# OpenDriveLab/ST-P3

Hardware: AMD Instinct MI355X
Metric: BEV samples/sec (6-cam x 3-frame fwd+bwd) (higher is better)
Workload: dtype bf16 convs / f32 voxel pool; 1 GPU; BASELINE configs[2]: batch=4/GPU, 6-cam 224x480, T=3, full STP3 fwd+bwd with segmentation + pedestrian + hdmap + depth CE + instance centerness/offset + flow losses, grad-clip 5, Adam; EfficientNet-B4, D=48, C=64, BEV 200x200; global_batch=4, parallelism=dp1, launch=hipgraph

## Files before the change

### st-p3_amd/csrc/stp3_dwconv.hip

```cpp
#include <hip/hip_runtime.h>
#include <mutex>
#include <vector>
#include <stdint.h>
#include <stdlib.h>

#include "stp3_cdna.h"
#include "stp3_hip.h"

namespace {

struct DwDims {
    int N, H, W, C, Ho, Wo;
    int pad_t, pad_l;
};

template <typename T> struct Vec;
template <> struct Vec<float> {
    static constexpr int N = 4;
    float4 v;
    __device__ void load(const float* p) { v = *reinterpret_cast<const float4*>(p); }
    __device__ void store(float* p) const { *reinterpret_cast<float4*>(p) = v; }
    __device__ void zero() { v = make_float4(0.f, 0.f, 0.f, 0.f); }
    __device__ void to_float(float* f) const { f[0] = v.x; f[1] = v.y; f[2] = v.z; f[3] = v.w; }
    __device__ void from_float(const float* f) { v = make_float4(f[0], f[1], f[2], f[3]); }
};
struct bf16x8 { uint4 v; };
template <> struct Vec<uint16_t> {
    static constexpr int N = 8;
    uint4 v;
    __device__ void load(const uint16_t* p) { v = *reinterpret_cast<const uint4*>(p); }
    __device__ void store(uint16_t* p) const { *reinterpret_cast<uint4*>(p) = v; }
    __device__ void zero() { v = make_uint4(0, 0, 0, 0); }
    __device__ void to_float(float* f) const {
        const uint32_t w[4] = {v.x, v.y, v.z, v.w};
#pragma unroll
        for (int i = 0; i < 4; ++i) {
            f[2 * i] = __uint_as_float(w[i] << 16);
            f[2 * i + 1] = __uint_as_float(w[i] & 0xffff0000u);
        }
    }
    __device__ void from_float(const float* f) {
        uint32_t w[4];
#pragma unroll
        for (int i = 0; i < 4; ++i) w[i] = pack_bf16(f[2 * i], f[2 * i + 1]);
        v = make_uint4(w[0], w[1], w[2], w[3]);
    }
};

template <typename T, typename Off>
__device__ __forceinline__ const T* at(const T* base, Off byte_off) {
    return reinterpret_cast<const T*>(reinterpret_cast<const char*>(base) + byte_off);
}
template <typename T, typename Off>
__device__ __forceinline__ T* at(T* base, Off byte_off) {
    return reinterpret_cast<T*>(reinterpret_cast<char*>(base) + byte_off);
}

__device__ __forceinline__ int xcd_order(int bid, int nwg) {
    const int q = nwg >> 3, r = nwg & 7, xcd = bid & 7;
    return (xcd < r ? xcd * (q + 1) : r * (q + 1) + (xcd - r) * q) + (bid >> 3);
}

template <typename T, int K, int S, int TW, bool FLIP, typename Off, bool AFFINE = false>
__global__ __launch_bounds__(256) void dwconv_fwd_kernel(DwDims d, const T* __restrict__ x,
                                                         const float* __restrict__ w, const float* __restrict__ bias,
                                                         T* __restrict__ y, const float* __restrict__ coef = nullptr,
                                                         int act = STP3_ACT_NONE) {
    constexpr int VN = Vec<T>::N;
    const int CV = d.C / VN;
    const int wgroups = (d.Wo + TW - 1) / TW;
    const Off total = (Off)d.N * d.Ho * wgroups * CV;
    const Off tid = (Off)xcd_order(blockIdx.x, gridDim.x) * 256 + threadIdx.x;
    if (tid >= total) return;
    const int cv = (int)(tid % (Off)CV);
    Off r = tid / (Off)CV;
    const int wg = (int)(r % (Off)wgroups);
    r /= (Off)wgroups;
    const int ho = (int)(r % (Off)d.Ho);
    const int n = (int)(r / (Off)d.Ho);
    const int c0 = cv * VN;
    const int wo0 = wg * TW;
    float acc[TW][VN];
#pragma unroll
    for (int i = 0; i < TW; ++i)
#pragma unroll
        for (int j = 0; j < VN; ++j) acc[i][j] = bias ? bias[c0 + j] : 0.f;
    constexpr int SPAN = (TW - 1) * S + K;
    const int wi0 = wo0 * S - d.pad_l;
    const Off pix = (Off)d.C * sizeof(T);
    const Off wtap = (Off)d.C * sizeof(float);
    const Off wc0 = (Off)c0 * sizeof(float);
#pragma unroll
    for (int kh = 0; kh < K; ++kh) {
        const int hi = ho * S + kh - d.pad_t;
        if (hi < 0 || hi >= d.H) continue;
        float wk[K][VN];
#pragma unroll
        for (int kw = 0; kw < K; ++kw) {
            const float* wp = at(w, (Off)(FLIP ? (K - 1 - kh) * K + (K - 1 - kw) : kh * K + kw) * wtap + wc0);
#pragma unroll
            for (int j = 0; j < VN; ++j) wk[kw][j] = wp[j];
        }
        const Off xrow = ((Off)(n * d.H + hi) * d.W) * pix + (Off)c0 * sizeof(T);
        float xin[SPAN][VN];
#pragma unroll
        for (int i = 0; i < SPAN; ++i) {
            const int wi = wi0 + i;
            Vec<T> v;
            if (wi >= 0 && wi < d.W) v.load(at(x, xrow + (Off)wi * pix)); else v.zero();
            v.to_float(xin[i]);
        }
#pragma unroll
        for (int o = 0; o < TW; ++o)
#pragma unroll
            for (int kw = 0; kw < K; ++kw)
#pragma unroll
                for (int j = 0; j < VN; ++j) acc[o][j] = fmaf(xin[o * S + kw][j], wk[kw][j], acc[o][j]);
    }
    const Off yrow = ((Off)(n * d.Ho + ho) * d.Wo) * pix + (Off)c0 * sizeof(T);
    float cs[VN], ct[VN];
    if (AFFINE) {
#pragma unroll
        for (int j = 0; j < VN; ++j) {
            cs[j] = coef[c0 + j];
            ct[j] = coef[d.C + c0 + j];
        }
    }
#pragma unroll
    for (int o = 0; o < TW; ++o) {
        if (wo0 + o < d.Wo) {
            Vec<T> v;
            v.from_float(acc[o]);
            if (AFFINE) {
                float t[VN];
                v.to_float(t);
#pragma unroll
                for (int j = 0; j < VN; ++j) t[j] = fmaf(t[j], cs[j], ct[j]);
                if (act == STP3_ACT_SWISH) {
#pragma unroll
                    for (int j = 0; j < VN; ++j) t[j] = t[j] * fast_sigmoid(t[j]);
                } else if (act == STP3_ACT_RELU) {
#pragma unroll
                    for (int j = 0; j < VN; ++j) t[j] = fmaxf(t[j], 0.f);
                }
                v.from_float(t);
            }
            v.store(at(y, yrow + (Off)(wo0 + o) * pix));
        }
    }
}

template <typename T, int K>
__global__ __launch_bounds__(256) void dwconv_bwd_data_s2_kernel(DwDims d, int qrows, int qcols, const T* __restrict__ dy,
                                                                 const float* __restrict__ w, T* __restrict__ dx) {
    constexpr int VN = Vec<T>::N;
    constexpr int R = (K + 1) / 2;
    constexpr bool kRegW = K == 3;
    const int CV = d.C / VN;
    const int CVB = min(CV, 256);
    const int QL = 256 / CVB;
    const int cv = blockIdx.y * CVB + threadIdx.x % CVB, ql = threadIdx.x / CVB;
    if (ql >= QL || cv >= CV) return;
    const int c0 = cv * VN;
    float wr[kRegW ? K * K : 1][VN];
    if (kRegW) {
#pragma unroll
        for (int t = 0; t < K * K; ++t)
#pragma unroll
            for (int j = 0; j < VN; ++j) wr[t][j] = w[t * d.C + c0 + j];
    }
    const int a0 = d.pad_t >> 1, b0 = d.pad_l >> 1;
    const int64_t total = (int64_t)d.N * qrows * qcols;
    for (int64_t q = (int64_t)blockIdx.x * QL + ql; q < total; q += (int64_t)gridDim.x * QL) {
        const int bi = (int)(q % qcols);
        int64_t r = q / qcols;
        const int ai = (int)(r % qrows);
        const int n = (int)(r / qrows);
        const int a = a0 + ai, b = b0 + bi;
        float acc[2][2][VN];
#pragma unroll
        for (int pr = 0; pr < 2; ++pr)
#pragma unroll
            for (int pc = 0; pc < 2; ++pc)
#pragma unroll
                for (int j = 0; j < VN; ++j) acc[pr][pc][j] = 0.f;
#pragma unroll
        for (int dr = 0; dr < R; ++dr) {
            const int ho = a - dr;
            if (ho < 0 || ho >= d.Ho) continue;
#pragma unroll
            for (int dc = 0; dc < R; ++dc) {
                const int wo = b - dc;
                if (wo < 0 || wo >= d.Wo) continue;
                Vec<T> v;
                v.load(dy + ((int64_t)(n * d.Ho + ho) * d.Wo + wo) * d.C + c0);
                float g[VN];
                v.to_float(g);
#pragma unroll
                for (int pr = 0; pr < 2; ++pr) {
                    const int kh = 2 * dr + pr;
                    if (kh >= K) continue;
#pragma unroll
                    for (int pc = 0; pc < 2; ++pc) {
                        const int kw = 2 * dc + pc;
                        if (kw >= K) continue;
                        if (kRegW) {
#pragma unroll
                            for (int j = 0; j < VN; ++j) acc[pr][pc][j] = fmaf(g[j], wr[kh * K + kw][j], acc[pr][pc][j]);
                        } else {
#pragma unroll
                            for (int j = 0; j < VN; ++j)
                                acc[pr][pc][j] = fmaf(g[j], w[(kh * K + kw) * d.C + c0 + j], acc[pr][pc][j]);
                        }
                    }
                }
            }
        }
#pragma unroll
        for (int pr = 0; pr < 2; ++pr) {
            const int hi = 2 * a + pr - d.pad_t;
            if (hi < 0 || hi >= d.H) continue;
#pragma unroll
            for (int pc = 0; pc < 2; ++pc) {
                const int wi = 2 * b + pc - d.pad_l;
                if (wi < 0 || wi >= d.W) continue;
                Vec<T> o;
                o.from_float(acc[pr][pc]);
                o.store(dx + ((int64_t)(n * d.H + hi) * d.W + wi) * d.C + c0);
            }
        }
    }
}

template <typename T, int K, int S, typename Off>
__global__ __launch_bounds__(256) void dwconv_bwd_weight_kernel(DwDims d, int nbx, const T* __restrict__ x,
                                                                const T* __restrict__ dy,
                                                                float* __restrict__ partial) {
    constexpr int VN = Vec<T>::N;
    constexpr int KK = K * K;
    constexpr int TW = 4;
    constexpr int SPAN = (TW - 1) * S + K;
    extern __shared__ __attribute__((aligned(16))) float red[];
    const int CV = d.C / VN;
    const int CVB = min(CV, 256);
    const int PL = 256 / CVB;
    const int cvb = threadIdx.x % CVB, pl = threadIdx.x / CVB;
    const int v = xcd_order(blockIdx.x, gridDim.x);
    const int kh = v % K;
    const int bxi = (v / K) % nbx, byi = v / (K * nbx);
    const int cv = byi * CVB + cvb;
    const bool live = pl < PL && cv < CV;
    const int c0 = cv * VN;
    float acc[K][VN];
#pragma unroll
    for (int t = 0; t < K; ++t)
#pragma unroll
        for (int j = 0; j < VN; ++j) acc[t][j] = 0.f;
    const int wgroups = (d.Wo + TW - 1) / TW;
    const int ngroups = d.N * d.Ho * wgroups;
    if (live) {
        for (int p = bxi * PL + pl; p < ngroups; p += nbx * PL) {
            const int wg = p % wgroups;
            const int r = p / wgroups;
            const int ho = r % d.Ho;
            const int n = r / d.Ho;
            const int hi = ho * S + kh - d.pad_t;
            if (hi < 0 || hi >= d.H) continue;
            const int wo0 = wg * TW;
            const Off pix = (Off)d.C * sizeof(T);
            const Off grow = ((Off)(n * d.Ho + ho) * d.Wo + wo0) * pix + (Off)c0 * sizeof(T);
            const Off xrow = ((Off)(n * d.H + hi) * d.W) * pix + (Off)c0 * sizeof(T);
            const int wi0 = wo0 * S - d.pad_l;
            float g[TW][VN], xin[SPAN][VN];
#pragma unroll
            for (int o = 0; o < TW; ++o) {
                Vec<T> v;
                if (wo0 + o < d.Wo) v.load(at(dy, grow + (Off)o * pix)); else v.zero();
                v.to_float(g[o]);
            }
#pragma unroll
            for (int i = 0; i < SPAN; ++i) {
                const int wi = wi0 + i;
                Vec<T> v;
                if (wi >= 0 && wi < d.W) v.load(at(x, xrow + (Off)wi * pix)); else v.zero();
                v.to_float(xin[i]);
            }
#pragma unroll
            for (int o = 0; o < TW; ++o)
#pragma unroll
                for (int kw = 0; kw < K; ++kw)
#pragma unroll
                    for (int j = 0; j < VN; ++j) acc[kw][j] = fmaf(g[o][j], xin[o * S + kw][j], acc[kw][j]);
        }
    }
    const int rowlen = CVB * VN;
    if (pl < PL) {
#pragma unroll
        for (int t = 0; t < K; ++t)
#pragma unroll
            for (int j = 0; j < VN; ++j) red[(pl * K + t) * rowlen + cvb * VN + j] = acc[t][j];
    }
    __syncthreads();
    for (int i = threadIdx.x; i < K * rowlen; i += 256) {
        const int t = i / rowlen, cc = i % rowlen;
        const int c = byi * rowlen + cc;
        if (c >= d.C) continue;
        float s = 0.f;
        for (int q = 0; q < PL; ++q) s += red[(q * K + t) * rowlen + cc];
        partial[((int64_t)bxi * KK + kh * K + t) * d.C + c] = s;
    }
}

__global__ __launch_bounds__(256) void dwconv_reduce_partials_kernel(int nblocks, int n, const float* __restrict__ partial,
                                                                     float* __restrict__ dw, int channels) {
    __shared__ float red[256];
    const int il = threadIdx.x & 63, bl = threadIdx.x >> 6;
    const int i = blockIdx.x * 64 + il;
    float s0 = 0.f, s1 = 0.f, s2 = 0.f, s3 = 0.f;
    if (i < n) {
        int b = bl;
        for (; b + 12 < nblocks; b += 16) {
            const float a = partial[(int64_t)b * n + i], c = partial[(int64_t)(b + 4) * n + i];
            const float e = partial[(int64_t)(b + 8) * n + i], f = partial[(int64_t)(b + 12) * n + i];
            s0 += a; s1 += c; s2 += e; s3 += f;
        }
        for (; b < nblocks; b += 4) s0 += partial[(int64_t)b * n + i];
    }
    red[threadIdx.x] = (s0 + s1) + (s2 + s3);
    __syncthreads();
    if (bl == 0 && i < n) {
        const int o = channels > 0 ? (i % channels) * (n / channels) + i / channels : i;
        dw[o] = (red[il] + red[64 + il]) + (red[128 + il] + red[192 + il]);
    }
}


template <typename T, int K, int S, typename Off>
__global__ __launch_bounds__(256) void dwconv_fwd_stats_kernel(DwDims d, const T* __restrict__ x, const float* __restrict__ w,
                                                               T* __restrict__ y, float* __restrict__ partial) {
    constexpr int VN = Vec<T>::N;
    constexpr int TW = 4;
    constexpr int SPAN = (TW - 1) * S + K;
    extern __shared__ __attribute__((aligned(16))) float red[];
    const int CV = d.C / VN;
    const int CVB = min(CV, 256);
    const int PL = 256 / CVB;
    const int cvb = threadIdx.x % CVB, pl = threadIdx.x / CVB;
    const int cv = blockIdx.y * CVB + cvb;
    const bool live = pl < PL && cv < CV;
    const int c0 = cv * VN;
    float s1[VN], s2[VN];
#pragma unroll
    for (int j = 0; j < VN; ++j) s1[j] = s2[j] = 0.f;
    const int wgroups = (d.Wo + TW - 1) / TW;
    const int ngroups = d.N * d.Ho * wgroups;
    if (live) {
        for (int p = blockIdx.x * PL + pl; p < ngroups; p += gridDim.x * PL) {
            const int wg = p % wgroups;
            const int r = p / wgroups;
            const int ho = r % d.Ho;
            const int n = r / d.Ho;
            const int wo0 = wg * TW;
            float acc[TW][VN];
#pragma unroll
            for (int i = 0; i < TW; ++i)
#pragma unroll
                for (int j = 0; j < VN; ++j) acc[i][j] = 0.f;
            const int wi0 = wo0 * S - d.pad_l;
            const Off pix = (Off)d.C * sizeof(T);
            const Off wtap = (Off)d.C * sizeof(float), wc0 = (Off)c0 * sizeof(float);
#pragma unroll
            for (int kh = 0; kh < K; ++kh) {
                const int hi = ho * S + kh - d.pad_t;
                if (hi < 0 || hi >= d.H) continue;
                float wk[K][VN];
#pragma unroll
                for (int kw = 0; kw < K; ++kw) {
                    const float* wp = at(w, (Off)(kh * K + kw) * wtap + wc0);
#pragma unroll
                    for (int j = 0; j < VN; ++j) wk[kw][j] = wp[j];
                }
                const Off xrow = ((Off)(n * d.H + hi) * d.W) * pix + (Off)c0 * sizeof(T);
                float xin[SPAN][VN];
#pragma unroll
                for (int i = 0; i < SPAN; ++i) {
                    const int wi = wi0 + i;
                    Vec<T> v;
                    if (wi >= 0 && wi < d.W) v.load(at(x, xrow + (Off)wi * pix)); else v.zero();
                    v.to_float(xin[i]);
                }
#pragma unroll
                for (int o = 0; o < TW; ++o)
#pragma unroll
                    for (int kw = 0; kw < K; ++kw)
#pragma unroll
                        for (int j = 0; j < VN; ++j) acc[o][j] = fmaf(xin[o * S + kw][j], wk[kw][j], acc[o][j]);
            }
            const Off yrow = ((Off)(n * d.Ho + ho) * d.Wo) * pix + (Off)c0 * sizeof(T);
#pragma unroll
            for (int o = 0; o < TW; ++o) {
                if (wo0 + o < d.Wo) {
                    Vec<T> v;
                    v.from_float(acc[o]);
                    v.store(at(y, yrow + (Off)(wo0 + o) * pix));
                    float rv[VN];
                    v.to_float(rv);
#pragma unroll
                    for (int j = 0; j < VN; ++j) {
                        s1[j] += rv[j];
                        s2[j] = fmaf(rv[j], rv[j], s2[j]);
                    }
                }
            }
        }
    }
    const int rowlen = CVB * VN;
    if (pl < PL) {
#pragma unroll
        for (int j = 0; j < VN; ++j) {
            red[(pl * 2) * rowlen + cvb * VN + j] = live ? s1[j] : 0.f;
            red[(pl * 2 + 1) * rowlen + cvb * VN + j] = live ? s2[j] : 0.f;
        }
    }
    __syncthreads();
    for (int i = threadIdx.x; i < 2 * rowlen; i += 256) {
        const int k = i / rowlen, cc = i - k * rowlen;
        const int c = blockIdx.y * rowlen + cc;
        if (c >= d.C) continue;
        float t = 0.f;
        for (int q = 0; q < PL; ++q) t += red[(q * 2 + k) * rowlen + cc];
        partial[((int64_t)blockIdx.x * 2 + k) * d.C + c] = t;
    }
}

constexpr int kRedCols = 8, kRedLanes = 256 / kRedCols;
__global__ __launch_bounds__(256) void dwconv_stat_reduce_kernel(int nblocks, int n, const float* __restrict__ partial,
                                                                 float* __restrict__ sums) {
    __shared__ double red[256];
    const int il = threadIdx.x % kRedCols, bl = threadIdx.x / kRedCols;
    const int i = blockIdx.x * kRedCols + il;
    double s0 = 0.0, s1 = 0.0, s2 = 0.0, s3 = 0.0;
    if (i < n) {
        const float* src = partial + i;
        int b = bl;
        for (; b + 3 * kRedLanes < nblocks; b += 4 * kRedLanes) {
            const float a = src[(int64_t)b * n], c = src[(int64_t)(b + kRedLanes) * n];
            const float e = src[(int64_t)(b + 2 * kRedLanes) * n], f = src[(int64_t)(b + 3 * kRedLanes) * n];
            s0 += (double)a; s1 += (double)c; s2 += (double)e; s3 += (double)f;
        }
        for (; b < nblocks; b += kRedLanes) s0 += (double)src[(int64_t)b * n];
    }
    red[threadIdx.x] = (s0 + s1) + (s2 + s3);
    __syncthreads();
    for (int st = kRedLanes / 2; st > 0; st >>= 1) {
        if (bl < st) red[threadIdx.x] += red[threadIdx.x + st * kRedCols];
        __syncthreads();
    }
    if (bl == 0 && i < n) sums[i] = (float)red[il];
}

struct BnFin {
    float inv_count, unbias, eps, momentum;
    const float* gamma;
    const float* beta;
    float* running_mean;
    float* running_var;
    float* coef;
};
__global__ __launch_bounds__(256) void dwconv_stat_reduce_finalize_kernel(int nblocks, int C, const float* __restrict__ partial,
                                                                          float* __restrict__ sums, BnFin f) {
    __shared__ double red[256];
    const int il = threadIdx.x % kRedCols, bl = threadIdx.x / kRedCols;
    const int c = blockIdx.x * (kRedCols / 2) + (il & 3), k = il >> 2;
    const int n = 2 * C;
    const int i = k * C + c;
    double s0 = 0.0, s1 = 0.0, s2 = 0.0, s3 = 0.0;
    if (c < C) {
        const float* src = partial + i;
        int b = bl;
        for (; b + 3 * kRedLanes < nblocks; b += 4 * kRedLanes) {
            const float a = src[(int64_t)b * n], cc = src[(int64_t)(b + kRedLanes) * n];
            const float e = src[(int64_t)(b + 2 * kRedLanes) * n], g = src[(int64_t)(b + 3 * kRedLanes) * n];
            s0 += (double)a; s1 += (double)cc; s2 += (double)e; s3 += (double)g;
        }
        for (; b < nblocks; b += kRedLanes) s0 += (double)src[(int64_t)b * n];
    }
    red[threadIdx.x] = (s0 + s1) + (s2 + s3);
    __syncthreads();
    for (int st = kRedLanes / 2; st > 0; st >>= 1) {
        if (bl < st) red[threadIdx.x] += red[threadIdx.x + st * kRedCols];
        __syncthreads();
    }
    if (bl == 0 && c < C) sums[i] = (float)red[il];
    if (threadIdx.x < 4 && c < C) {
        const float sum = (float)red[il], sq = (float)red[4 + il];
        const float mean = sum * f.inv_count;
        const float var = fmaxf(sq * f.inv_count - mean * mean, 0.f);
        const float invstd = 1.0f / sqrtf(var + f.eps);
        const float scale = (f.gamma ? f.gamma[c] : 1.f) * invstd;
        f.coef[c] = scale;
        f.coef[C + c] = (f.beta ? f.beta[c] : 0.f) - mean * scale;
        f.coef[2 * C + c] = mean;
        f.coef[3 * C + c] = invstd;
        if (f.running_mean) {
            f.running_mean[c] = (1.f - f.momentum) * f.running_mean[c] + f.momentum * mean;
            f.running_var[c] = (1.f - f.momentum) * f.running_var[c] + f.momentum * var * f.unbias;
        }
    }
}

constexpr int kStatBlocks = 2048;
constexpr int kWgradBlocks = 512;

template <typename Kern>
inline int resident_blocks(Kern kernel, size_t lds) {
    struct Entry { const void* fn; size_t lds; int blocks; };
    static std::mutex mu;
    static std::vector<Entry> cache;
    static int cus = 0;
    std::lock_guard<std::mutex> lock(mu);
    for (const Entry& e : cache)
        if (e.fn == (const void*)kernel && e.lds == lds) return e.blocks;
    if (cus == 0) {
        int dev = 0;
        if (hipGetDevice(&dev) != hipSuccess ||
            hipDeviceGetAttribute(&cus, hipDeviceAttributeMultiprocessorCount, dev) != hipSuccess || cus < 1)
            cus = 256;
    }
    int per_cu = 0;
    if (hipOccupancyMaxActiveBlocksPerMultiprocessor(&per_cu, kernel, 256, lds) != hipSuccess || per_cu < 1) per_cu = 1;
    cache.push_back(Entry{(const void*)kernel, lds, per_cu * cus});
    return per_cu * cus;
}

inline int status() {
    hipError_t e = hipGetLastError();
    return e == hipSuccess ? STP3_OK : -(int)e;
}

inline int check(const stp3_dwconv_dims* p, DwDims* d, int* vec) {
    if (!p) return STP3_EINVAL;
    if (p->N <= 0 || p->H <= 0 || p->W <= 0 || p->C <= 0 || p->Ho <= 0 || p->Wo <= 0) return STP3_EINVAL;
    if (!(((p->K == 3 || p->K == 5) && (p->stride == 1 || p->stride == 2)) || (p->K == 7 && p->stride == 1)))
        return STP3_EUNSUP;
    if (p->dtype != STP3_DTYPE_F32 && p->dtype != STP3_DTYPE_BF16) return STP3_EUNSUP;
    *vec = p->dtype == STP3_DTYPE_BF16 ? 8 : 4;
    if (p->C % *vec) return STP3_EUNSUP;
    if ((int64_t)p->N * p->H * p->W * p->C >= (1LL << 40)) return STP3_EUNSUP;
    d->N = p->N; d->H = p->H; d->W = p->W; d->C = p->C; d->Ho = p->Ho; d->Wo = p->Wo;
    d->pad_t = p->pad_top; d->pad_l = p->pad_left;
    return STP3_OK;
}

template <typename T>
inline bool small_tensors(const DwDims& d) {
    const uint64_t lim = (1ull << 32) - (uint64_t)(d.W + d.Wo + 16) * d.C * sizeof(float);
    return (uint64_t)d.N * d.H * d.W * d.C * sizeof(T) < lim && (uint64_t)d.N * d.Ho * d.Wo * d.C * sizeof(T) < lim &&
           (uint64_t)64 * d.C * sizeof(float) < lim;
}

template <typename T, int K, int S>
int launch_fwd(const DwDims& d, const void* x, const float* w, const float* bias, void* y, hipStream_t s) {
    constexpr int TW = 4;
    const int CV = d.C / Vec<T>::N;
    const int64_t total = (int64_t)d.N * d.Ho * ((d.Wo + TW - 1) / TW) * CV;
    if (small_tensors<T>(d))
        hipLaunchKernelGGL((dwconv_fwd_kernel<T, K, S, TW, false, uint32_t>), dim3((unsigned)((total + 255) / 256)), dim3(256), 0,
                           s, d, (const T*)x, w, bias, (T*)y, (const float*)nullptr, 0);
    else
        hipLaunchKernelGGL((dwconv_fwd_kernel<T, K, S, TW, false, uint64_t>), dim3((unsigned)((total + 255) / 256)), dim3(256), 0,
                           s, d, (const T*)x, w, bias, (T*)y, (const float*)nullptr, 0);
    return status();
}
template <int K, int S>
int launch_fwd_affine(const DwDims& d, const void* x, const float* w, const float* coef, int act, void* y, hipStream_t s) {
    typedef uint16_t T;
    constexpr int TW = 4;
    const int CV = d.C / Vec<T>::N;
    const int64_t total = (int64_t)d.N * d.Ho * ((d.Wo + TW - 1) / TW) * CV;
    if (small_tensors<T>(d))
        hipLaunchKernelGGL((dwconv_fwd_kernel<T, K, S, TW, false, uint32_t, true>), dim3((unsigned)((total + 255) / 256)), dim3(256),
                           0, s, d, (const T*)x, w, (const float*)nullptr, (T*)y, coef, act);
    else
        hipLaunchKernelGGL((dwconv_fwd_kernel<T, K, S, TW, false, uint64_t, true>), dim3((unsigned)((total + 255) / 256)), dim3(256),
                           0, s, d, (const T*)x, w, (const float*)nullptr, (T*)y, coef, act);
    return status();
}
template <typename T, int K, int S>
int launch_fwd_stats(const DwDims& d, const void* x, const float* w, void* y, float* sums, float* ws, hipStream_t s,
                     const BnFin* fin = nullptr) {
    constexpr int VN = Vec<T>::N;
    const int CV = d.C / VN;
    const int CVB = CV < 256 ? CV : 256;
    const int PL = 256 / CVB;
    const int64_t ngroups = (int64_t)d.N * d.Ho * ((d.Wo + 3) / 4);
    if (ngroups >= (1LL << 31)) return STP3_EUNSUP;
    const int by = (CV + CVB - 1) / CVB;
    int64_t want = (ngroups + PL - 1) / PL;
    const size_t lds = (size_t)PL * 2 * CVB * VN * sizeof(float);
    const bool small = small_tensors<T>(d);
    int limit = small ? resident_blocks(dwconv_fwd_stats_kernel<T, K, S, uint32_t>, lds)
                      : resident_blocks(dwconv_fwd_stats_kernel<T, K, S, uint64_t>, lds);
    if (limit > kStatBlocks) limit = kStatBlocks;
    const int cap = limit / by > 0 ? limit / by : 1;
    const int bx = (int)(want < cap ? want : cap);
    if (small)
        hipLaunchKernelGGL((dwconv_fwd_stats_kernel<T, K, S, uint32_t>), dim3(bx, by), dim3(256), lds, s, d, (const T*)x, w, (T*)y, ws);
    else
        hipLaunchKernelGGL((dwconv_fwd_stats_kernel<T, K, S, uint64_t>), dim3(bx, by), dim3(256), lds, s, d, (const T*)x, w, (T*)y, ws);
    if (fin)
        hipLaunchKernelGGL(dwconv_stat_reduce_finalize_kernel, dim3((d.C + kRedCols / 2 - 1) / (kRedCols / 2)), dim3(256), 0, s, bx,
                           d.C, ws, sums, *fin);
    else
        hipLaunchKernelGGL(dwconv_stat_reduce_kernel, dim3((2 * d.C + kRedCols - 1) / kRedCols), dim3(256), 0, s, bx, 2 * d.C, ws, sums);
    return status();
}
template <typename T, int K, int S>
int launch_bwd_data(const DwDims& d, const void* dy, const float* w, void* dx, hipStream_t s) {
    if constexpr (S == 1) {
        constexpr int TW = 4;
        DwDims f = d;
        f.H = d.Ho; f.W = d.Wo; f.Ho = d.H; f.Wo = d.W;
        f.pad_t = K - 1 - d.pad_t; f.pad_l = K - 1 - d.pad_l;
        const int64_t n = (int64_t)f.N * f.Ho * ((f.Wo + TW - 1) / TW) * (f.C / Vec<T>::N);
        if (small_tensors<T>(f))
            hipLaunchKernelGGL((dwconv_fwd_kernel<T, K, 1, TW, true, uint32_t>), dim3((unsigned)((n + 255) / 256)), dim3(256), 0, s,
                               f, (const T*)dy, w, (const float*)nullptr, (T*)dx, (const float*)nullptr, 0);
        else
            hipLaunchKernelGGL((dwconv_fwd_kernel<T, K, 1, TW, true, uint64_t>), dim3((unsigned)((n + 255) / 256)), dim3(256), 0, s,
                               f, (const T*)dy, w, (const float*)nullptr, (T*)dx, (const float*)nullptr, 0);
        return status();
    } else if constexpr (S == 2) {
        const int qrows = ((d.H - 1 + d.pad_t) >> 1) - (d.pad_t >> 1) + 1;
        const int qcols = ((d.W - 1 + d.pad_l) >> 1) - (d.pad_l >> 1) + 1;
        const int CV = d.C / Vec<T>::N;
        const int CVB = CV < 256 ? CV : 256;
        const int QL = 256 / CVB;
        const int by = (CV + CVB - 1) / CVB;
        const int64_t want = ((int64_t)d.N * qrows * qcols + QL - 1) / QL;
        int cap = resident_blocks(dwconv_bwd_data_s2_kernel<T, K>, 0) / by;
        if (cap < 1) cap = 1;
        const int bx = (int)(want < cap ? want : cap);
        hipLaunchKernelGGL((dwconv_bwd_data_s2_kernel<T, K>), dim3(bx, by), dim3(256), 0, s, d, qrows, qcols, (const T*)dy, w,
                           (T*)dx);
        return status();
    } else {
        return STP3_EUNSUP;
    }
}
template <typename T, int K, int S>
int launch_bwd_weight(const DwDims& d, const void* x, const void* dy, float* dw, float* ws, hipStream_t s, bool param_layout) {
    constexpr int VN = Vec<T>::N;
    const int CV = d.C / VN;
    const int CVB = CV < 256 ? CV : 256;
    const int PL = 256 / CVB;
    const int64_t npix = (int64_t)d.N * d.Ho * ((d.Wo + 3) / 4);
    if (npix >= (1LL << 31)) return STP3_EUNSUP;
    int64_t want = (npix + PL - 1) / PL;
    const int by = (CV + CVB - 1) / CVB;
    const size_t lds = (size_t)PL * K * CVB * VN * sizeof(float);
    const bool small = small_tensors<T>(d);
    int cap = (small ? resident_blocks(dwconv_bwd_weight_kernel<T, K, S, uint32_t>, lds)
                     : resident_blocks(dwconv_bwd_weight_kernel<T, K, S, uint64_t>, lds)) / (by * K);
    if (cap > kWgradBlocks) cap = kWgradBlocks;
    if (cap < 1) cap = 1;
    const int bx = (int)(want < cap ? want : cap);
    if (small)
        hipLaunchKernelGGL((dwconv_bwd_weight_kernel<T, K, S, uint32_t>), dim3(bx * by * K), dim3(256), lds, s, d, bx, (const T*)x,
                           (const T*)dy, ws);
    else
        hipLaunchKernelGGL((dwconv_bwd_weight_kernel<T, K, S, uint64_t>), dim3(bx * by * K), dim3(256), lds, s, d, bx, (const T*)x,
                           (const T*)dy, ws);
    const int n = K * K * d.C;
    hipLaunchKernelGGL(dwconv_reduce_partials_kernel, dim3((n + 63) / 64), dim3(256), 0, s, bx, n, ws, dw, param_layout ? d.C : 0);
    return status();
}

#define DISPATCH(FN, ...)                                                                               \
    do {                                                                                                \
        const bool bf = p->dtype == STP3_DTYPE_BF16;                                                    \
        if (p->K == 3 && p->stride == 1) return bf ? FN<uint16_t, 3, 1>(__VA_ARGS__) : FN<float, 3, 1>(__VA_ARGS__); \
        if (p->K == 3 && p->stride == 2) return bf ? FN<uint16_t, 3, 2>(__VA_ARGS__) : FN<float, 3, 2>(__VA_ARGS__); \
        if (p->K == 5 && p->stride == 1) return bf ? FN<uint16_t, 5, 1>(__VA_ARGS__) : FN<float, 5, 1>(__VA_ARGS__); \
        if (p->K == 7) return bf ? FN<uint16_t, 7, 1>(__VA_ARGS__) : FN<float, 7, 1>(__VA_ARGS__);                   \
        return bf ? FN<uint16_t, 5, 2>(__VA_ARGS__) : FN<float, 5, 2>(__VA_ARGS__);                       \
    } while (0)

}

extern "C" {

int stp3_dwconv2d_fwd(const stp3_dwconv_dims* p, const void* x, const float* w, void* y, void* stream) {
    DwDims d; int vec;
    int rc = check(p, &d, &vec);
    if (rc) return rc;
    if (!x || !w || !y) return STP3_EINVAL;
    DISPATCH(launch_fwd, d, x, w, (const float*)nullptr, y, (hipStream_t)stream);
}

int stp3_dwconv2d_fwd_bias(const stp3_dwconv_dims* p, const void* x, const float* w, const float* bias, void* y,
                           void* stream) {
    DwDims d; int vec;
    int rc = check(p, &d, &vec);
    if (rc) return rc;
    if (!x || !w || !y) return STP3_EINVAL;
    DISPATCH(launch_fwd, d, x, w, bias, y, (hipStream_t)stream);
}

int stp3_dwconv2d_fwd_affine(const stp3_dwconv_dims* p, const void* x, const float* w, const float* coef, int32_t act,
                             void* y, void* stream) {
    DwDims d; int vec;
    int rc = check(p, &d, &vec);
    if (rc) return rc;
    if (!x || !w || !coef || !y) return STP3_EINVAL;
    if (act != STP3_ACT_NONE && act != STP3_ACT_RELU && act != STP3_ACT_SWISH) return STP3_EINVAL;
    if (p->dtype != STP3_DTYPE_BF16 || p->K == 7) return STP3_EUNSUP;
    hipStream_t s = (hipStream_t)stream;
    if (p->K == 3) return p->stride == 1 ? launch_fwd_affine<3, 1>(d, x, w, coef, act, y, s) : launch_fwd_affine<3, 2>(d, x, w, coef, act, y, s);
    return p->stride == 1 ? launch_fwd_affine<5, 1>(d, x, w, coef, act, y, s) : launch_fwd_affine<5, 2>(d, x, w, coef, act, y, s);
}

int stp3_dwconv2d_fwd_stats_workspace(const stp3_dwconv_dims* p, size_t* bytes) {
    DwDims d; int vec;
    int rc = check(p, &d, &vec);
    if (rc) return rc;
    if (!bytes) return STP3_EINVAL;
    *bytes = (size_t)kStatBlocks * 2 * p->C * sizeof(float);
    return STP3_OK;
}

int stp3_dwconv2d_fwd_stats(const stp3_dwconv_dims* p, const void* x, const float* w, void* y, float* sums, void* workspace,
                            size_t workspace_bytes, void* stream) {
    DwDims d; int vec;
    int rc = check(p, &d, &vec);
    if (rc) return rc;
    if (!x || !w || !y || !sums || !workspace) return STP3_EINVAL;
    if (workspace_bytes < (size_t)kStatBlocks * 2 * p->C * sizeof(float)) return STP3_ENOSPACE;
    DISPATCH(launch_fwd_stats, d, x, w, y, sums, (float*)workspace, (hipStream_t)stream);
}

int stp3_dwconv2d_fwd_stats_bn(const stp3_dwconv_dims* p, const void* x, const float* w, void* y, float* sums, double count,
                               const float* gamma, const float* beta, float eps, float momentum, float* running_mean,
                               float* running_var, float* coef, void* workspace, size_t workspace_bytes, void* stream) {
    DwDims d; int vec;
    int rc = check(p, &d, &vec);
    if (rc) return rc;
    if (!x || !w || !y || !sums || !coef || !workspace || !(count >= 1.0)) return STP3_EINVAL;
    if ((running_mean == nullptr) != (running_var == nullptr)) return STP3_EINVAL;
    if (workspace_bytes < (size_t)kStatBlocks * 2 * p->C * sizeof(float)) return STP3_ENOSPACE;
    BnFin fin;
    fin.inv_count = (float)(1.0 / count);
    fin.unbias = count > 1.0 ? (float)(count / (count - 1.0)) : 1.f;
    fin.eps = eps; fin.momentum = momentum; fin.gamma = gamma; fin.beta = beta;
    fin.running_mean = running_mean; fin.running_var = running_var; fin.coef = coef;
    DISPATCH(launch_fwd_stats, d, x, w, y, sums, (float*)workspace, (hipStream_t)stream, &fin);
}

int stp3_dwconv2d_bwd_data(const stp3_dwconv_dims* p, const void* dy, const float* w, void* dx, void* stream) {
    DwDims d; int vec;
    int rc = check(p, &d, &vec);
    if (rc) return rc;
    if (!dy || !w || !dx) return STP3_EINVAL;
    DISPATCH(launch_bwd_data, d, dy, w, dx, (hipStream_t)stream);
}

int stp3_dwconv2d_bwd_weight_workspace(const stp3_dwconv_dims* p, size_t* bytes) {
    DwDims d; int vec;
    int rc = check(p, &d, &vec);
    if (rc) return rc;
    if (!bytes) return STP3_EINVAL;
    *bytes = (size_t)kWgradBlocks * p->K * p->K * p->C * sizeof(float);
    return STP3_OK;
}

int stp3_dwconv2d_bwd_weight(const stp3_dwconv_dims* p, const void* x, const void* dy, float* dw, void* workspace,
                             size_t workspace_bytes, void* stream) {
    DwDims d; int vec;
    int rc = check(p, &d, &vec);
    if (rc) return rc;
    if (!x || !dy || !dw || !workspace) return STP3_EINVAL;
    if (workspace_bytes < (size_t)kWgradBlocks * p->K * p->K * p->C * sizeof(float)) return STP3_ENOSPACE;
    DISPATCH(launch_bwd_weight, d, x, dy, dw, (float*)workspace, (hipStream_t)stream, false);
}

int stp3_dwconv2d_bwd_weight_oihw(const stp3_dwconv_dims* p, const void* x, const void* dy, float* dw, void* workspace,
                                  size_t workspace_bytes, void* stream) {
    DwDims d; int vec;
    int rc = check(p, &d, &vec);
    if (rc) return rc;
    if (!x || !dy || !dw || !workspace) return STP3_EINVAL;
    if (workspace_bytes < (size_t)kWgradBlocks * p->K * p->K * p->C * sizeof(float)) return STP3_ENOSPACE;
    DISPATCH(launch_bwd_weight, d, x, dy, dw, (float*)workspace, (hipStream_t)stream, true);
}

}
```

Baseline: 113.3 samples/s.

## Use buffer loads for depthwise conv and stage stride-2 bwd taps in LDS

Adds a BufAddr offset mode for tensors under 2 GiB. In it, the forward, forward-stats and weight-gradient depthwise kernels read through buffer_load16 with out-of-bounds offsets that hardware zero-fills, replacing branchy global loads and 64-bit address math. Separately, the stride-2 backward-data kernel for K>3 now stages its weights in LDS as float4 slabs and re-splits channels across the y grid instead of reading weights from global memory per tap. This adds LDS usage and a block barrier, and relies on buffer descriptor bounds being correct.

```diff
diff --git a/st-p3_amd/csrc/stp3_dwconv.hip b/st-p3_amd/csrc/stp3_dwconv.hip
--- a/st-p3_amd/csrc/stp3_dwconv.hip
+++ b/st-p3_amd/csrc/stp3_dwconv.hip
@@ -61,23 +61,49 @@
     return (xcd < r ? xcd * (q + 1) : r * (q + 1) + (xcd - r) * q) + (bid >> 3);
 }
 
+struct BufAddr {};
+template <typename Off> struct OffsetOf { typedef Off type; };
+template <> struct OffsetOf<BufAddr> { typedef uint32_t type; };
+template <typename Off> struct IsBuf { static constexpr bool value = false; };
+template <> struct IsBuf<BufAddr> { static constexpr bool value = true; };
+
+template <typename T, int SPAN, typename Off>
+__device__ __forceinline__ void load_span(float (*xin)[Vec<T>::N], const T* __restrict__ x, stp3_buffer xb,
+                                          typename OffsetOf<Off>::type xrow, typename OffsetOf<Off>::type pix, int wi0, int W) {
+    typedef typename OffsetOf<Off>::type O;
+    O off = xrow + (O)wi0 * pix;
+#pragma unroll
+    for (int i = 0; i < SPAN; ++i, off += pix) {
+        const int wi = wi0 + i;
+        Vec<T> v;
+        if constexpr (IsBuf<Off>::value) {
+            const stp3_u32x4 q = buffer_load16(xb, (unsigned)wi < (unsigned)W ? off : (O)kBufOob);
+            __builtin_memcpy(&v.v, &q, 16);
+        } else {
+            if (wi >= 0 && wi < W) v.load(at(x, off)); else v.zero();
+        }
+        v.to_float(xin[i]);
+    }
+}
+
 template <typename T, int K, int S, int TW, bool FLIP, typename Off, bool AFFINE = false>
 __global__ __launch_bounds__(256) void dwconv_fwd_kernel(DwDims d, const T* __restrict__ x,
                                                          const float* __restrict__ w, const float* __restrict__ bias,
                                                          T* __restrict__ y, const float* __restrict__ coef = nullptr,
                                                          int act = STP3_ACT_NONE) {
     constexpr int VN = Vec<T>::N;
+    typedef typename OffsetOf<Off>::type O;
     const int CV = d.C / VN;
     const int wgroups = (d.Wo + TW - 1) / TW;
-    const Off total = (Off)d.N * d.Ho * wgroups * CV;
-    const Off tid = (Off)xcd_order(blockIdx.x, gridDim.x) * 256 + threadIdx.x;
+    const O total = (O)d.N * d.Ho * wgroups * CV;
+    const O tid = (O)xcd_order(blockIdx.x, gridDim.x) * 256 + threadIdx.x;
     if (tid >= total) return;
-    const int cv = (int)(tid % (Off)CV);
-    Off r = tid / (Off)CV;
-    const int wg = (int)(r % (Off)wgroups);
-    r /= (Off)wgroups;
-    const int ho = (int)(r % (Off)d.Ho);
-    const int n = (int)(r / (Off)d.Ho);
+    const int cv = (int)(tid % (O)CV);
+    O r = tid / (O)CV;
+    const int wg = (int)(r % (O)wgroups);
+    r /= (O)wgroups;
+    const int ho = (int)(r % (O)d.Ho);
+    const int n = (int)(r / (O)d.Ho);
     const int c0 = cv * VN;
     const int wo0 = wg * TW;
     float acc[TW][VN];
@@ -87,9 +113,10 @@
         for (int j = 0; j < VN; ++j) acc[i][j] = bias ? bias[c0 + j] : 0.f;
     constexpr int SPAN = (TW - 1) * S + K;
     const int wi0 = wo0 * S - d.pad_l;
-    const Off pix = (Off)d.C * sizeof(T);
-    const Off wtap = (Off)d.C * sizeof(float);
-    const Off wc0 = (Off)c0 * sizeof(float);
+    const O pix = (O)d.C * sizeof(T);
+    const O wtap = (O)d.C * sizeof(float);
+    const O wc0 = (O)c0 * sizeof(float);
+    const stp3_buffer xb = make_buffer(x, IsBuf<Off>::value ? (uint32_t)d.N * d.H * d.W * (uint32_t)pix : 0u);
 #pragma unroll
     for (int kh = 0; kh < K; ++kh) {
         const int hi = ho * S + kh - d.pad_t;
@@ -97,19 +124,13 @@
         float wk[K][VN];
 #pragma unroll
         for (int kw = 0; kw < K; ++kw) {
-            const float* wp = at(w, (Off)(FLIP ? (K - 1 - kh) * K + (K - 1 - kw) : kh * K + kw) * wtap + wc0);
+            const float* wp = at(w, (O)(FLIP ? (K - 1 - kh) * K + (K - 1 - kw) : kh * K + kw) * wtap + wc0);
 #pragma unroll
             for (int j = 0; j < VN; ++j) wk[kw][j] = wp[j];
         }
-        const Off xrow = ((Off)(n * d.H + hi) * d.W) * pix + (Off)c0 * sizeof(T);
+        const O xrow = ((O)(n * d.H + hi) * d.W) * pix + (O)c0 * sizeof(T);
         float xin[SPAN][VN];
-#pragma unroll
-        for (int i = 0; i < SPAN; ++i) {
-            const int wi = wi0 + i;
-            Vec<T> v;
-            if (wi >= 0 && wi < d.W) v.load(at(x, xrow + (Off)wi * pix)); else v.zero();
-            v.to_float(xin[i]);
-        }
+        load_span<T, SPAN, Off>(xin, x, xb, xrow, pix, wi0, d.W);
 #pragma unroll
         for (int o = 0; o < TW; ++o)
 #pragma unroll
@@ -117,7 +138,7 @@
 #pragma unroll
                 for (int j = 0; j < VN; ++j) acc[o][j] = fmaf(xin[o * S + kw][j], wk[kw][j], acc[o][j]);
     }
-    const Off yrow = ((Off)(n * d.Ho + ho) * d.Wo) * pix + (Off)c0 * sizeof(T);
+    const O yrow = ((O)(n * d.Ho + ho) * d.Wo) * pix + (O)c0 * sizeof(T);
     float cs[VN], ct[VN];
     if (AFFINE) {
 #pragma unroll
@@ -145,22 +166,39 @@
                 }
                 v.from_float(t);
             }
-            v.store(at(y, yrow + (Off)(wo0 + o) * pix));
-        }
-    }
+            v.store(at(y, yrow + (O)(wo0 + o) * pix));
+        }
+    }
+}
+
+__host__ __device__ constexpr int quad_slab(int K) { return K == 3 ? 256 : 32; }
+
+template <int VN, int KK, int SLAB>
+__device__ __forceinline__ void stage_taps(float* tab, const float* __restrict__ w, int C, int CVB) {
+    const int cbase = blockIdx.y * CVB * VN;
+    for (int t = 0; t < KK; ++t) {
+        const float* src = w + t * C + cbase;
+        for (int cl = threadIdx.x; cl < CVB * VN; cl += 256)
+            tab[((t * (VN / 4) + (cl % VN) / 4) * SLAB + cl / VN) * 4 + (cl & 3)] = cbase + cl < C ? src[cl] : 0.f;
+    }
+    __syncthreads();
 }
 
 template <typename T, int K>
 __global__ __launch_bounds__(256) void dwconv_bwd_data_s2_kernel(DwDims d, int qrows, int qcols, const T* __restrict__ dy,
                                                                  const float* __restrict__ w, T* __restrict__ dx) {
-    constexpr int VN = Vec<T>::N;
+    constexpr int VN = Vec<T>::N, HV = VN / 4, SLAB = quad_slab(K);
     constexpr int R = (K + 1) / 2;
     constexpr bool kRegW = K == 3;
+    extern __shared__ __attribute__((aligned(16))) float taps[];
     const int CV = d.C / VN;
-    const int CVB = min(CV, 256);
+    const int CVB = (CV + gridDim.y - 1) / gridDim.y;
     const int QL = 256 / CVB;
-    const int cv = blockIdx.y * CVB + threadIdx.x % CVB, ql = threadIdx.x / CVB;
+    const int cvb = threadIdx.x % CVB;
+    const int cv = blockIdx.y * CVB + cvb, ql = threadIdx.x / CVB;
+    if (!kRegW) stage_taps<VN, K * K, SLAB>(taps, w, d.C, CVB);
     if (ql >= QL || cv >= CV) return;
+    const float4* tp = reinterpret_cast<const float4*>(taps) + cvb;
     const int c0 = cv * VN;
     float wr[kRegW ? K * K : 1][VN];
     if (kRegW) {
@@ -208,9 +246,14 @@
 #pragma unroll
                             for (int j = 0; j < VN; ++j) acc[pr][pc][j] = fmaf(g[j], wr[kh * K + kw][j], acc[pr][pc][j]);
                         } else {
-#pragma unroll
-                            for (int j = 0; j < VN; ++j)
-                                acc[pr][pc][j] = fmaf(g[j], w[(kh * K + kw) * d.C + c0 + j], acc[pr][pc][j]);
+                            float wt[VN];
+#pragma unroll
+                            for (int h = 0; h < HV; ++h) {
+                                const float4 t = tp[((kh * K + kw) * HV + h) * SLAB];
+                                wt[4 * h] = t.x; wt[4 * h + 1] = t.y; wt[4 * h + 2] = t.z; wt[4 * h + 3] = t.w;
+                            }
+#pragma unroll
+                            for (int j = 0; j < VN; ++j) acc[pr][pc][j] = fmaf(g[j], wt[j], acc[pr][pc][j]);
                         }
                     }
                 }
@@ -240,6 +283,8 @@
     constexpr int KK = K * K;
     constexpr int TW = 4;
     constexpr int SPAN = (TW - 1) * S + K;
+    constexpr bool BUF = IsBuf<Off>::value;
+    typedef typename OffsetOf<Off>::type O;
     extern __shared__ __attribute__((aligned(16))) float red[];
     const int CV = d.C / VN;
     const int CVB = min(CV, 256);
@@ -259,6 +304,9 @@
     const int wgroups = (d.Wo + TW - 1) / TW;
     const int ngroups = d.N * d.Ho * wgroups;
     if (live) {
+        const O pix = (O)d.C * sizeof(T);
+        const stp3_buffer xb = make_buffer(x, BUF ? (uint32_t)d.N * d.H * d.W * (uint32_t)pix : 0u);
+        const stp3_buffer gb = make_buffer(dy, BUF ? (uint32_t)d.N * d.Ho * d.Wo * (uint32_t)pix : 0u);
         for (int p = bxi * PL + pl; p < ngroups; p += nbx * PL) {
             const int wg = p % wgroups;
             const int r = p / wgroups;
@@ -267,22 +315,32 @@
             const int hi = ho * S + kh - d.pad_t;
             if (hi < 0 || hi >= d.H) continue;
             const int wo0 = wg * TW;
-            const Off pix = (Off)d.C * sizeof(T);
-            const Off grow = ((Off)(n * d.Ho + ho) * d.Wo + wo0) * pix + (Off)c0 * sizeof(T);
-            const Off xrow = ((Off)(n * d.H + hi) * d.W) * pix + (Off)c0 * sizeof(T);
+            const O grow = ((O)(n * d.Ho + ho) * d.Wo + wo0) * pix + (O)c0 * sizeof(T);
+            const O xrow = ((O)(n * d.H + hi) * d.W) * pix + (O)c0 * sizeof(T);
             const int wi0 = wo0 * S - d.pad_l;
             float g[TW][VN], xin[SPAN][VN];
-#pragma unroll
-            for (int o = 0; o < TW; ++o) {
+            O goff = grow, xoff = xrow + (O)wi0 * pix;
+#pragma unroll
+            for (int o = 0; o < TW; ++o, goff += pix) {
                 Vec<T> v;
-                if (wo0 + o < d.Wo) v.load(at(dy, grow + (Off)o * pix)); else v.zero();
+                if constexpr (BUF) {
+                    const stp3_u32x4 q = buffer_load16(gb, wo0 + o < d.Wo ? goff : (O)kBufOob);
+                    __builtin_memcpy(&v.v, &q, 16);
+                } else {
+                    if (wo0 + o < d.Wo) v.load(at(dy, goff)); else v.zero();
+                }
                 v.to_float(g[o]);
             }
 #pragma unroll
-            for (int i = 0; i < SPAN; ++i) {
+            for (int i = 0; i < SPAN; ++i, xoff += pix) {
                 const int wi = wi0 + i;
                 Vec<T> v;
-                if (wi >= 0 && wi < d.W) v.load(at(x, xrow + (Off)wi * pix)); else v.zero();
+                if constexpr (BUF) {
+                    const stp3_u32x4 q = buffer_load16(xb, (unsigned)wi < (unsigned)d.W ? xoff : (O)kBufOob);
+                    __builtin_memcpy(&v.v, &q, 16);
+                } else {
+                    if (wi >= 0 && wi < d.W) v.load(at(x, xoff)); else v.zero();
+                }
                 v.to_float(xin[i]);
             }
 #pragma unroll
@@ -341,6 +399,7 @@
     constexpr int VN = Vec<T>::N;
     constexpr int TW = 4;
     constexpr int SPAN = (TW - 1) * S + K;
+    typedef typename OffsetOf<Off>::type O;
     extern __shared__ __attribute__((aligned(16))) float red[];
     const int CV = d.C / VN;
     const int CVB = min(CV, 256);
@@ -355,6 +414,9 @@
     const int wgroups = (d.Wo + TW - 1) / TW;
     const int ngroups = d.N * d.Ho * wgroups;
     if (live) {
+        const O pix = (O)d.C * sizeof(T);
+        const O wtap = (O)d.C * sizeof(float), wc0 = (O)c0 * sizeof(float);
+        const stp3_buffer xb = make_buffer(x, IsBuf<Off>::value ? (uint32_t)d.N * d.H * d.W * (uint32_t)pix : 0u);
         for (int p = blockIdx.x * PL + pl; p < ngroups; p += gridDim.x * PL) {
             const int wg = p % wgroups;
             const int r = p / wgroups;
@@ -367,8 +429,6 @@
 #pragma unroll
                 for (int j = 0; j < VN; ++j) acc[i][j] = 0.f;
             const int wi0 = wo0 * S - d.pad_l;
-            const Off pix = (Off)d.C * sizeof(T);
-            const Off wtap = (Off)d.C * sizeof(float), wc0 = (Off)c0 * sizeof(float);
 #pragma unroll
             for (int kh = 0; kh < K; ++kh) {
                 const int hi = ho * S + kh - d.pad_t;
@@ -376,19 +436,13 @@
                 float wk[K][VN];
 #pragma unroll
                 for (int kw = 0; kw < K; ++kw) {
-                    const float* wp = at(w, (Off)(kh * K + kw) * wtap + wc0);
+                    const float* wp = at(w, (O)(kh * K + kw) * wtap + wc0);
 #pragma unroll
                     for (int j = 0; j < VN; ++j) wk[kw][j] = wp[j];
                 }
-                const Off xrow = ((Off)(n * d.H + hi) * d.W) * pix + (Off)c0 * sizeof(T);
+                const O xrow = ((O)(n * d.H + hi) * d.W) * pix + (O)c0 * sizeof(T);
                 float xin[SPAN][VN];
-#pragma unroll
-                for (int i = 0; i < SPAN; ++i) {
-                    const int wi = wi0 + i;
-                    Vec<T> v;
-                    if (wi >= 0 && wi < d.W) v.load(at(x, xrow + (Off)wi * pix)); else v.zero();
-                    v.to_float(xin[i]);
-                }
+                load_span<T, SPAN, Off>(xin, x, xb, xrow, pix, wi0, d.W);
 #pragma unroll
                 for (int o = 0; o < TW; ++o)
 #pragma unroll
@@ -396,13 +450,13 @@
 #pragma unroll
                         for (int j = 0; j < VN; ++j) acc[o][j] = fmaf(xin[o * S + kw][j], wk[kw][j], acc[o][j]);
             }
-            const Off yrow = ((Off)(n * d.Ho + ho) * d.Wo) * pix + (Off)c0 * sizeof(T);
+            const O yrow = ((O)(n * d.Ho + ho) * d.Wo) * pix + (O)c0 * sizeof(T);
 #pragma unroll
             for (int o = 0; o < TW; ++o) {
                 if (wo0 + o < d.Wo) {
                     Vec<T> v;
                     v.from_float(acc[o]);
-                    v.store(at(y, yrow + (Off)(wo0 + o) * pix));
+                    v.store(at(y, yrow + (O)(wo0 + o) * pix));
                     float rv[VN];
                     v.to_float(rv);
 #pragma unroll
@@ -559,32 +613,36 @@
            (uint64_t)64 * d.C * sizeof(float) < lim;
 }
 
+template <typename T>
+inline bool buffer_tensors(const DwDims& d) {
+    const uint64_t lim = 1ull << 31;
+    return (uint64_t)d.N * d.H * d.W * d.C * sizeof(T) < lim && (uint64_t)d.N * d.Ho * d.Wo * d.C * sizeof(T) < lim;
+}
+
+template <typename T, int K, int S, bool FLIP, bool AFFINE>
+int launch_tiles(const DwDims& d, const void* x, const float* w, const float* bias, void* y, const float* coef, int act,
+                 hipStream_t s) {
+    constexpr int TW = 4;
+    const int64_t total = (int64_t)d.N * d.Ho * ((d.Wo + TW - 1) / TW) * (d.C / Vec<T>::N);
+    const dim3 grid((unsigned)((total + 255) / 256));
+    if (buffer_tensors<T>(d))
+        hipLaunchKernelGGL((dwconv_fwd_kernel<T, K, S, TW, FLIP, BufAddr, AFFINE>), grid, dim3(256), 0, s, d, (const T*)x, w, bias,
+                           (T*)y, coef, act);
+    else if (small_tensors<T>(d))
+        hipLaunchKernelGGL((dwconv_fwd_kernel<T, K, S, TW, FLIP, uint32_t, AFFINE>), grid, dim3(256), 0, s, d, (const T*)x, w, bias,
+                           (T*)y, coef, act);
+    else
+        hipLaunchKernelGGL((dwconv_fwd_kernel<T, K, S, TW, FLIP, uint64_t, AFFINE>), grid, dim3(256), 0, s, d, (const T*)x, w, bias,
+                           (T*)y, coef, act);
+    return status();
+}
 template <typename T, int K, int S>
 int launch_fwd(const DwDims& d, const void* x, const float* w, const float* bias, void* y, hipStream_t s) {
-    constexpr int TW = 4;
-    const int CV = d.C / Vec<T>::N;
-    const int64_t total = (int64_t)d.N * d.Ho * ((d.Wo + TW - 1) / TW) * CV;
-    if (small_tensors<T>(d))
-        hipLaunchKernelGGL((dwconv_fwd_kernel<T, K, S, TW, false, uint32_t>), dim3((unsigned)((total + 255) / 256)), dim3(256), 0,
-                           s, d, (const T*)x, w, bias, (T*)y, (const float*)nullptr, 0);
-    else
-        hipLaunchKernelGGL((dwconv_fwd_kernel<T, K, S, TW, false, uint64_t>), dim3((unsigned)((total + 255) / 256)), dim3(256), 0,
-                           s, d, (const T*)x, w, bias, (T*)y, (const float*)nullptr, 0);
-    return status();
+    return launch_tiles<T, K, S, false, false>(d, x, w, bias, y, nullptr, 0, s);
 }
 template <int K, int S>
 int launch_fwd_affine(const DwDims& d, const void* x, const float* w, const float* coef, int act, void* y, hipStream_t s) {
-    typedef uint16_t T;
-    constexpr int TW = 4;
-    const int CV = d.C / Vec<T>::N;
-    const int64_t total = (int64_t)d.N * d.Ho * ((d.Wo + TW - 1) / TW) * CV;
-    if (small_tensors<T>(d))
-        hipLaunchKernelGGL((dwconv_fwd_kernel<T, K, S, TW, false, uint32_t, true>), dim3((unsigned)((total + 255) / 256)), dim3(256),
-                           0, s, d, (const T*)x, w, (const float*)nullptr, (T*)y, coef, act);
-    else
-        hipLaunchKernelGGL((dwconv_fwd_kernel<T, K, S, TW, false, uint64_t, true>), dim3((unsigned)((total + 255) / 256)), dim3(256),
-                           0, s, d, (const T*)x, w, (const float*)nullptr, (T*)y, coef, act);
-    return status();
+    return launch_tiles<uint16_t, K, S, false, true>(d, x, w, nullptr, y, coef, act, s);
 }
 template <typename T, int K, int S>
 int launch_fwd_stats(const DwDims& d, const void* x, const float* w, void* y, float* sums, float* ws, hipStream_t s,
@@ -596,18 +654,19 @@
     const int64_t ngroups = (int64_t)d.N * d.Ho * ((d.Wo + 3) / 4);
     if (ngroups >= (1LL << 31)) return STP3_EUNSUP;
     const int by = (CV + CVB - 1) / CVB;
-    int64_t want = (ngroups + PL - 1) / PL;
+    const int64_t want = (ngroups + PL - 1) / PL;
     const size_t lds = (size_t)PL * 2 * CVB * VN * sizeof(float);
-    const bool small = small_tensors<T>(d);
-    int limit = small ? resident_blocks(dwconv_fwd_stats_kernel<T, K, S, uint32_t>, lds)
-                      : resident_blocks(dwconv_fwd_stats_kernel<T, K, S, uint64_t>, lds);
-    if (limit > kStatBlocks) limit = kStatBlocks;
-    const int cap = limit / by > 0 ? limit / by : 1;
-    const int bx = (int)(want < cap ? want : cap);
-    if (small)
-        hipLaunchKernelGGL((dwconv_fwd_stats_kernel<T, K, S, uint32_t>), dim3(bx, by), dim3(256), lds, s, d, (const T*)x, w, (T*)y, ws);
-    else
-        hipLaunchKernelGGL((dwconv_fwd_stats_kernel<T, K, S, uint64_t>), dim3(bx, by), dim3(256), lds, s, d, (const T*)x, w, (T*)y, ws);
+    int bx = 0;
+    auto go = [&](auto kernel) {
+        int limit = resident_blocks(kernel, lds);
+        if (limit > kStatBlocks) limit = kStatBlocks;
+        const int cap = limit / by > 0 ? limit / by : 1;
+        bx = (int)(want < cap ? want : cap);
+        hipLaunchKernelGGL(kernel, dim3(bx, by), dim3(256), lds, s, d, (const T*)x, w, (T*)y, ws);
+    };
+    if (buffer_tensors<T>(d)) go(dwconv_fwd_stats_kernel<T, K, S, BufAddr>);
+    else if (small_tensors<T>(d)) go(dwconv_fwd_stats_kernel<T, K, S, uint32_t>);
+    else go(dwconv_fwd_stats_kernel<T, K, S, uint64_t>);
     if (fin)
         hipLaunchKernelGGL(dwconv_stat_reduce_finalize_kernel, dim3((d.C + kRedCols / 2 - 1) / (kRedCols / 2)), dim3(256), 0, s, bx,
                            d.C, ws, sums, *fin);
@@ -618,30 +677,23 @@
 template <typename T, int K, int S>
 int launch_bwd_data(const DwDims& d, const void* dy, const float* w, void* dx, hipStream_t s) {
     if constexpr (S == 1) {
-        constexpr int TW = 4;
         DwDims f = d;
         f.H = d.Ho; f.W = d.Wo; f.Ho = d.H; f.Wo = d.W;
         f.pad_t = K - 1 - d.pad_t; f.pad_l = K - 1 - d.pad_l;
-        const int64_t n = (int64_t)f.N * f.Ho * ((f.Wo + TW - 1) / TW) * (f.C / Vec<T>::N);
-        if (small_tensors<T>(f))
-            hipLaunchKernelGGL((dwconv_fwd_kernel<T, K, 1, TW, true, uint32_t>), dim3((unsigned)((n + 255) / 256)), dim3(256), 0, s,
-                               f, (const T*)dy, w, (const float*)nullptr, (T*)dx, (const float*)nullptr, 0);
-        else
-            hipLaunchKernelGGL((dwconv_fwd_kernel<T, K, 1, TW, true, uint64_t>), dim3((unsigned)((n + 255) / 256)), dim3(256), 0, s,
-                               f, (const T*)dy, w, (const float*)nullptr, (T*)dx, (const float*)nullptr, 0);
-        return status();
+        return launch_tiles<T, K, 1, true, false>(f, dy, w, nullptr, dx, nullptr, 0, s);
     } else if constexpr (S == 2) {
         const int qrows = ((d.H - 1 + d.pad_t) >> 1) - (d.pad_t >> 1) + 1;
         const int qcols = ((d.W - 1 + d.pad_l) >> 1) - (d.pad_l >> 1) + 1;
         const int CV = d.C / Vec<T>::N;
-        const int CVB = CV < 256 ? CV : 256;
+        const int by = (CV + quad_slab(K) - 1) / quad_slab(K);
+        const int CVB = (CV + by - 1) / by;
         const int QL = 256 / CVB;
-        const int by = (CV + CVB - 1) / CVB;
+        const size_t lds = K == 3 ? 0 : (size_t)K * K * Vec<T>::N * quad_slab(K) * sizeof(float);
         const int64_t want = ((int64_t)d.N * qrows * qcols + QL - 1) / QL;
-        int cap = resident_blocks(dwconv_bwd_data_s2_kernel<T, K>, 0) / by;
+        int cap = resident_blocks(dwconv_bwd_data_s2_kernel<T, K>, lds) / by;
         if (cap < 1) cap = 1;
         const int bx = (int)(want < cap ? want : cap);
-        hipLaunchKernelGGL((dwconv_bwd_data_s2_kernel<T, K>), dim3(bx, by), dim3(256), 0, s, d, qrows, qcols, (const T*)dy, w,
+        hipLaunchKernelGGL((dwconv_bwd_data_s2_kernel<T, K>), dim3(bx, by), dim3(256), lds, s, d, qrows, qcols, (const T*)dy, w,
                            (T*)dx);
         return status();
     } else {
@@ -665,12 +717,13 @@
     if (cap > kWgradBlocks) cap = kWgradBlocks;
     if (cap < 1) cap = 1;
     const int bx = (int)(want < cap ? want : cap);
-    if (small)
-        hipLaunchKernelGGL((dwconv_bwd_weight_kernel<T, K, S, uint32_t>), dim3(bx * by * K), dim3(256), lds, s, d, bx, (const T*)x,
-                           (const T*)dy, ws);
+    const dim3 grid(bx * by * K);
+    if (buffer_tensors<T>(d))
+        hipLaunchKernelGGL((dwconv_bwd_weight_kernel<T, K, S, BufAddr>), grid, dim3(256), lds, s, d, bx, (const T*)x, (const T*)dy, ws);
+    else if (small)
+        hipLaunchKernelGGL((dwconv_bwd_weight_kernel<T, K, S, uint32_t>), grid, dim3(256), lds, s, d, bx, (const T*)x, (const T*)dy, ws);
     else
-        hipLaunchKernelGGL((dwconv_bwd_weight_kernel<T, K, S, uint64_t>), dim3(bx * by * K), dim3(256), lds, s, d, bx, (const T*)x,
-                           (const T*)dy, ws);
+        hipLaunchKernelGGL((dwconv_bwd_weight_kernel<T, K, S, uint64_t>), grid, dim3(256), lds, s, d, bx, (const T*)x, (const T*)dy, ws);
     const int n = K * K * d.C;
     hipLaunchKernelGGL(dwconv_reduce_partials_kernel, dim3((n + 63) / 64), dim3(256), 0, s, bx, n, ws, dw, param_layout ? d.C : 0);
     return status();
```

Result: no change. 113.8 samples/s, median of 6 (+0.5%).
